# DakeQQ/Text-to-Speech-TTS-ONNX

Measured on AMD Instinct MI355X. Metric: audio_seconds_per_second, higher is better.
Workload: dtype f32

## Files before the change

text-to-speech-tts-onnx_amd/csrc/attention.hip:

```cpp
#include "common.h"
#include <functional>
#include <map>
#include <mutex>
#include <tuple>
#include "mfma.h"
#include "f5_kernels.h"
#include "x3_split.h"
#include "lds_dma.h"
#include <type_traits>
#include <string>
#include <algorithm>

namespace mi {

#define ATTN_XCD_MAP                                                                          \
    int bx_ = (int)blockIdx.x, by_ = (int)blockIdx.y;                                         \
    if (xmap) {                                                                               \
        const int l2 = bx_ + (int)gridDim.x * by_, slot = l2 >> 3;                            \
        by_ = (l2 & 7) + 8 * (slot / (int)gridDim.x);                                         \
        bx_ = slot % (int)gridDim.x;                                                          \
    }

#define ATTN_VARLEN_PROLOGUE                                                                  \
    const int NL = VARLEN ? lens[(bh / H) >> 1] : N;                                          \
// ... 390 lines not shown
}
__device__ __forceinline__ void attn_tr_use(attn_u2& d) {
#if defined(__HIP_DEVICE_COMPILE__)
    asm volatile("" : "+v"(d));
#endif
}
template <int N, int I = 0, typename F> __device__ __forceinline__ void attn_unroll(F&& f) {
    if constexpr (I < N) { f(std::integral_constant<int, I>{}); attn_unroll<N, I + 1>(f); }
}
template <int NP, int PLB, int S2> __device__ __forceinline__ void attn_v_tr_read(attn_u2 (&t)[2][NP][2], unsigned a0, unsigned a1) {
    attn_unroll<NP>([&](auto PL) {
        constexpr int pl = NP - 1 - decltype(PL)::value, o = pl * PLB + S2 * 16 * 128;
        attn_lds_rd64_tr16<o>(t[0][pl][0], a0); attn_lds_rd64_tr16<o + 8 * 128>(t[0][pl][1], a0);
        attn_lds_rd64_tr16<o>(t[1][pl][0], a1); attn_lds_rd64_tr16<o + 8 * 128>(t[1][pl][1], a1);
    });
}
#if defined(MI355TTS_ATTN_TRACE)
#define TSTAMP(v) do { __builtin_amdgcn_sched_barrier(0); asm volatile("s_memtime %0\n\ts_waitcnt lgkmcnt(0)" : "=s"(v) :: "memory"); __builtin_amdgcn_sched_barrier(0); } while (0)
#define TACC(k, t1, t0) tr_[k] += (t1) - (t0)
#else
#define TSTAMP(v) do { } while (0)
#define TACC(k, t1, t0) do { } while (0)
#endif
template <bool SPLIT2, bool KVP = false, int NP = 3, bool VARLEN = false, bool VROWS = false>
__global__ __launch_bounds__(256, NP == 2 ? 3 : 2) void attn_x3f_kernel(const float* __restrict__ q, const float* __restrict__ k,
                                                       const float* __restrict__ v, float* __restrict__ o, int H, int N,
                                                       float* __restrict__ ws, int* __restrict__ cnt,
                                                       unsigned char* __restrict__ o_planes, int o_np, int xmap = 0,
                                                       int cut1 = 0, int cut2 = 0, int cut3 = 0, const int* __restrict__ lens = nullptr) {
    ATTN_XCD_MAP
    static_assert(NP == 3 || (NP == 2 && KVP), "attn_x3f: the two-plane form reads pre-split K / V");
    static_assert(!VROWS || KVP, "attn_x3f: V as rows is a layout of the pre-split planes");
    using MF = std::conditional_t<NP == 3, Mfma<bf16>, Mfma<f16>>;
    using Frag = typename MF::Frag;
    constexpr int D = 64, KT = 64;
    constexpr int LDK = D + 8, LDV = VROWS ? D : KT + 4;
    constexpr int KPL = KT * LDK, VPL = VROWS ? KT * LDV : D * LDV;
    static_assert((NP * KPL * 2) % 16 == 0 && (VPL * 2) % 16 == 0, "attn_x3f: 16-byte aligned V planes");
    __shared__ __attribute__((aligned(16))) bf16 smem[NP * KPL + NP * VPL];
    static_assert(sizeof(smem) >= (2 * 32 * 64 + 2 * 64 * 2 + 4) * sizeof(float), "merge buffer fits the stage");
    bf16* Ks = smem;
    bf16* Vs = smem + NP * KPL;

    const int tid = threadIdx.x, wave = tid >> 6, lane = tid & 63, lr = lane & 31, hi = lane >> 5;
    const int bh = by_;
    ATTN_VARLEN_PROLOGUE
    const int q0 = SPLIT2 ? bx_ * 64 + (wave >> 1) * 32 : bx_ * 128 + wave * 32;
    const float* qb = q + (long)bh * N * D;
    const float* kb = k + (long)bh * N * D;
    const long vld = KVP ? (long)((N + 63) / 64 * 64) : (long)((N + 7) / 8 * 8);
    const float* vb = v + (long)bh * D * vld;
    const bf16* kpb = reinterpret_cast<const bf16*>(k) + (long)bh * NP * vld * D;
    const bf16* vpb = reinterpret_cast<const bf16*>(v) + (long)bh * NP * D * vld;

    auto split4 = [&](const float4 a, uint2& w1, uint2& w2, uint2& w3) __attribute__((always_inline)) {
        x3_split_pair(a.x, a.y, w1.x, w2.x, w3.x);
        x3_split_pair(a.z, a.w, w1.y, w2.y, w3.y);
    };
    auto split8 = [&](const float4 a, const float4 b, Frag& f1, Frag& f2, Frag& f3) __attribute__((always_inline)) {
        uint2 a1, a2, a3, b1, b2, b3;
        split4(a, a1, a2, a3); split4(b, b1, b2, b3);
        f1 = __builtin_bit_cast(Frag, u32x4{a1.x, a1.y, b1.x, b1.y});
// ... 94 lines not shown
                }
            }
        } else {
#pragma unroll
        for (int i = 0; i < 4; ++i) {
            const int vi = tid + i * 256;
            const int r = vi >> 4, c = vi & 15;
            uint2 w1, w2, w3;
            split4(kreg[i], w1, w2, w3);
            *reinterpret_cast<uint2*>(Ks + r * LDK + c * 4) = w1;
            *reinterpret_cast<uint2*>(Ks + KPL + r * LDK + c * 4) = w2;
            *reinterpret_cast<uint2*>(Ks + 2 * KPL + r * LDK + c * 4) = w3;
            split4(vreg[i], w1, w2, w3);
            *reinterpret_cast<uint2*>(Vs + r * LDV + c * 4) = w1;
            *reinterpret_cast<uint2*>(Vs + VPL + r * LDV + c * 4) = w2;
            *reinterpret_cast<uint2*>(Vs + 2 * VPL + r * LDV + c * 4) = w3;
        }
        }
    };

    unsigned vtr[2] = {0u, 0u};
    if constexpr (VROWS) {
        const int q4 = (lane >> 2) & 3;
        const unsigned a = lds_addr(Vs) + (4 * hi + q4) * (LDV * 2) + ((lane >> 4) & 1) * 32 + (lane & 3) * 8;
        vtr[0] = a + (q4 >> 1) * 64;
        vtr[1] = a + ((q4 >> 1) ^ 1) * 64;
    }
    f32x16 oacc[2];
#pragma unroll
    for (int r = 0; r < 16; ++r) { oacc[0][r] = 0.f; oacc[1][r] = 0.f; }
    float m_run = -INFINITY, l_run = 0.f;
#if defined(MI355TTS_ATTN_TRACE)
    unsigned long long tr_[8] = {0, 0, 0, 0, 0, 0, 0, 0}, ta_ = 0, tb_ = 0, tc_ = 0, td_ = 0, te_ = 0, tk_ = 0;
    TSTAMP(tk_);
#endif

    const int nstage_all = dead ? 0 : (NL + KT - 1) / KT;
    int st0 = (int)((long)blockIdx.z * nstage_all / gridDim.z);
    int nstage = (int)((long)(blockIdx.z + 1) * nstage_all / gridDim.z);
    if (cut1 > 0) {
        const int zz = (int)blockIdx.z, ZZ = (int)gridDim.z;
        st0 = zz == 0 ? 0 : zz == 1 ? cut1 : zz == 2 ? cut2 : cut3;
        nstage = zz + 1 == ZZ ? nstage_all : zz == 0 ? cut1 : zz == 1 ? cut2 : cut3;
    }
    if constexpr (VARLEN) { st0 = min(st0, nstage_all); nstage = min(nstage, nstage_all); }
    if (st0 < nstage) {
        load_regs(st0 * KT);
        store_lds();
        __syncthreads();
    }
    constexpr int TA[6] = {0, 1, 2, 0, 1, 0}, TB[6] = {2, 1, 0, 1, 0, 0};
    for (int st = st0; st < nstage; ++st) {
        if (st + 1 < nstage) load_regs((st + 1) * KT);
        auto tile = [&](int kt) {
            const int key0 = st * KT + kt * 32;
            TSTAMP(ta_);
            f32x16 sacc;
#pragma unroll
            for (int r = 0; r < 16; ++r) sacc[r] = 0.f;
#pragma unroll
            for (int ks = 0; ks < 4; ++ks) {
                Frag kf[NP];
#pragma unroll
                for (int pl = 0; pl < NP; ++pl)
                    kf[pl] = *reinterpret_cast<const Frag*>(Ks + pl * KPL + (kt * 32 + lr) * LDK + ks * 16 + hi * 8);
                if constexpr (NP == 3) {
#pragma unroll
                    for (int t = 0; t < 6; ++t) sacc = MF::mma(kf[TA[t]], qf3[ks][TB[t]], sacc);
                } else {
                    sacc = MF::mma(kf[1], qf3[ks][0], sacc);
                    sacc = MF::mma(kf[0], qf3[ks][1], sacc);
                    sacc = MF::mma(kf[0], qf3[ks][0], sacc);
                }
            }
            if (key0 + 32 > NL) {
#pragma unroll
                for (int r = 0; r < 16; ++r) {
                    const int key = key0 + (r & 3) + 8 * (r >> 2) + 4 * hi;
                    if (key >= NL) sacc[r] = -INFINITY;
                }
            }
            float mloc = -INFINITY;
#pragma unroll
            for (int r = 0; r < 16; ++r) mloc = fmaxf(mloc, sacc[r]);
            mloc = xor32_max(mloc);
#if defined(MI355TTS_ATTN_TRACE)
            { const float keep_ = mloc; asm volatile("" :: "v"(keep_)); }
#endif
            TSTAMP(tb_); TACC(0, tb_, ta_);
            float alpha = 1.f;
            if (!__all(mloc - m_run <= 8.0f)) {
                const float m_new = fmaxf(m_run, mloc);
                alpha = __builtin_amdgcn_exp2f(m_run - m_new);
                m_run = m_new;
#pragma unroll
                for (int r = 0; r < 16; ++r) { oacc[0][r] *= alpha; oacc[1][r] *= alpha; }
            }
            float p[16];
            float ls0 = 0.f, ls1 = 0.f;
#pragma unroll
            for (int r = 0; r < 16; r += 2) {
                float d0 = sacc[r] - m_run, d1 = sacc[r + 1] - m_run;
                asm("" : "+v"(d0)); asm("" : "+v"(d1));
                p[r] = __builtin_amdgcn_exp2f(d0); p[r + 1] = __builtin_amdgcn_exp2f(d1);
                ls0 += p[r]; ls1 += p[r + 1];
                asm("" : "+v"(ls0)); asm("" : "+v"(ls1));
            }
            float lsum = ls0 + ls1;
            lsum = xor32_sum(lsum);
            l_run = l_run * alpha + lsum;
#if defined(MI355TTS_ATTN_TRACE)
            { const float keep_ = l_run + p[0] + p[15]; asm volatile("" :: "v"(keep_)); }
#endif
            TSTAMP(tc_); TACC(1, tc_, tb_);
#pragma unroll
            for (int s2 = 0; s2 < 2; ++s2) {
                Frag pf[NP];
                if constexpr (NP == 3)
                    split8(float4{p[8 * s2], p[8 * s2 + 1], p[8 * s2 + 2], p[8 * s2 + 3]},
                           float4{p[8 * s2 + 4], p[8 * s2 + 5], p[8 * s2 + 6], p[8 * s2 + 7]}, pf[0], pf[1], pf[2]);
                else
                    split8p(float4{p[8 * s2], p[8 * s2 + 1], p[8 * s2 + 2], p[8 * s2 + 3]},
                            float4{p[8 * s2 + 4], p[8 * s2 + 5], p[8 * s2 + 6], p[8 * s2 + 7]}, pf[0], pf[1]);
                Frag vf[2][NP];
                if constexpr (VROWS) {
                    attn_u2 t[2][NP][2];
                    const unsigned a0 = vtr[0] + kt * (32 * LDV * 2), a1 = vtr[1] + kt * (32 * LDV * 2);
                    if (s2 == 0) attn_v_tr_read<NP, VPL * 2, 0>(t, a0, a1); else attn_v_tr_read<NP, VPL * 2, 1>(t, a0, a1);
                    attn_tr_wait();
#pragma unroll
                    for (int dt = 0; dt < 2; ++dt)
#pragma unroll
                        for (int pl = 0; pl < NP; ++pl) {
                            attn_tr_use(t[dt][pl][0]); attn_tr_use(t[dt][pl][1]);
                            vf[dt][pl] = __builtin_bit_cast(Frag, u32x4{t[dt][pl][0].x, t[dt][pl][0].y, t[dt][pl][1].x, t[dt][pl][1].y});
                        }
                } else {
#pragma unroll
                for (int dt = 0; dt < 2; ++dt)
#pragma unroll
                    for (int pl = 0; pl < NP; ++pl) {
                        const bf16* row = Vs + pl * VPL + (dt * 32 + lr) * LDV + kt * 32 + 16 * s2 + 4 * hi;
                        uint2 a2[2];
                        a2[0] = *reinterpret_cast<const uint2*>(row);
                        a2[1] = *reinterpret_cast<const uint2*>(row + 8);
                        vf[dt][pl] = __builtin_bit_cast(Frag, u32x4{a2[0].x, a2[0].y, a2[1].x, a2[1].y});
                    }
                }
                if constexpr (NP == 3) {
#pragma unroll
                    for (int t = 0; t < 6; ++t)
#pragma unroll
                        for (int dt = 0; dt < 2; ++dt) oacc[dt] = MF::mma(vf[dt][TA[t]], pf[TB[t]], oacc[dt]);
                } else {
                    oacc[0] = MF::mma(vf[0][1], pf[0], oacc[0]);
                    oacc[1] = MF::mma(vf[1][1], pf[0], oacc[1]);
                    oacc[0] = MF::mma(vf[0][0], pf[1], oacc[0]);
                    oacc[1] = MF::mma(vf[1][0], pf[1], oacc[1]);
                    oacc[0] = MF::mma(vf[0][0], pf[0], oacc[0]);
                    oacc[1] = MF::mma(vf[1][0], pf[0], oacc[1]);
                }
            }
            TSTAMP(td_); TACC(2, td_, tc_);
        };
        if constexpr (SPLIT2) {
            if (st * KT + (wave & 1) * 32 < NL) tile(wave & 1);
        } else {
#pragma unroll
            for (int kt = 0; kt < KT / 32; ++kt) {
                const int key0 = st * KT + kt * 32;
                if (key0 < NL) tile(kt);
            }
        }
        TSTAMP(ta_);
        __syncthreads();
        TSTAMP(tb_); TACC(3, tb_, ta_);
        if (st + 1 < nstage) {
            store_lds();
            TSTAMP(tc_); TACC(4, tc_, tb_);
            __syncthreads();
            TSTAMP(te_); TACC(5, te_, tc_);
        }
    }
#if defined(MI355TTS_ATTN_TRACE)
    TSTAMP(te_);
    if (blockIdx.x == 3 && blockIdx.y == 5 && (threadIdx.x & 63) == 0)
        printf("ATTN_TRACE z %d wave %d stages %d total %llu | S+max %llu exp %llu PV %llu bar1 %llu store %llu bar2 %llu\n", (int)blockIdx.z, wave, nstage - st0,
               te_ - tk_, tr_[0], tr_[1], tr_[2], tr_[3], tr_[4], tr_[5]);
#endif
    bool owner = true;
    constexpr int NG = SPLIT2 ? 2 : 4;
    int grp = wave;
    float* comb = reinterpret_cast<float*>(smem);
    float* stats = comb + 2 * 32 * 64;
    if constexpr (SPLIT2) {
        __syncthreads();
        grp = wave >> 1;
        owner = !(wave & 1);
        if (!owner) {
            stats[(grp * 64 + lane) * 2] = m_run; stats[(grp * 64 + lane) * 2 + 1] = l_run;
#pragma unroll
            for (int dt = 0; dt < 2; ++dt)
#pragma unroll
                for (int r = 0; r < 16; ++r) comb[((grp * 2 + dt) * 16 + r) * 64 + lane] = oacc[dt][r];
// ... 190 lines not shown
}

static int attn_pick_z(long units, long slot, int nstage, bool f32, int zmax, long ws_floats, long cnt_n) {
    auto fits = [&](int z) { return units * z * slot <= ws_floats && units <= cnt_n; };
    if (const int zf = opt(OPT_ATTN_Z_FORCE); zf > 0) return fits(zf) ? zf : 1;
    const int cus = device_cus();
    int Z = 1;
    double best = 1e30;
    for (int z = 1; z <= zmax; ++z) {
        if (z > 1 && (!fits(z) || nstage < 2 * z)) break;
        const double cost = (double)((units * z + cus - 1) / cus) / z * (1.0 + (f32 ? 0.09 : 0.06) * (z - 1));
        if (cost < best - 1e-9) { best = cost; Z = z; }
    }
    return Z;
}

struct AttnArgs { const AttnPlan& p; const void *q, *k, *v; void *o, *o_planes; int o_np; float* ws; int* cnt; const int* lens; hipStream_t s; };
using AttnThunk = void (*)(const AttnArgs&);
static dim3 attn_grid(const AttnPlan& p) { return dim3(p.grid[0], p.grid[1], p.grid[2]); }
template <typename T, bool SPLIT2, bool X3S, bool REFH, bool VARLEN> static void attn_go(const AttnArgs& a) {
    hipLaunchKernelGGL((attn_kernel<T, SPLIT2, X3S, REFH, VARLEN>), attn_grid(a.p), dim3(256), 0, a.s, (const T*)a.q, (const T*)a.k, (const T*)a.v,
                       (T*)a.o, a.p.H, a.p.N, a.ws, a.cnt, a.p.sscale, a.p.xmap, a.lens);
}
template <bool SPLIT2, bool KVP, int NP, bool VARLEN, bool VROWS> static void x3f_go(const AttnArgs& a) {
    hipLaunchKernelGGL((attn_x3f_kernel<SPLIT2, KVP, NP, VARLEN, VROWS>), attn_grid(a.p), dim3(256), 0, a.s, (const float*)a.q, (const float*)a.k,
                       (const float*)a.v, (float*)a.o, a.p.H, a.p.N, a.ws, a.cnt, (unsigned char*)a.o_planes, a.o_np, a.p.xmap, a.p.cut[0], a.p.cut[1],
                       a.p.cut[2], a.lens);
}
struct AttnEntry { const char* label; AttnThunk go[2][2]; };
#define ATTN_ROWS(T, SP, X3S, REFH) {{attn_go<T, SP, X3S, REFH, false>, nullptr}, {attn_go<T, SP, X3S, REFH, true>, nullptr}}
#define X3F_SPLITS(SP) {{x3f_go<SP, false, 3, false, false>, nullptr}, {x3f_go<SP, false, 3, true, false>, nullptr}}
#define X3F_PLANES(SP, NP) {{x3f_go<SP, true, NP, false, false>, x3f_go<SP, true, NP, false, true>}, {x3f_go<SP, true, NP, true, false>, x3f_go<SP, true, NP, true, true>}}
static const AttnEntry attn_table[ATTN_FORMS] = {
     {"attn_kernel<float, false>", ATTN_ROWS(float, false, false, false)},
     {"attn_kernel<float, true>", ATTN_ROWS(float, true, false, false)},
     {"attn_kernel<float, false, x3>", ATTN_ROWS(float, false, true, false)},
     {"attn_kernel<float, true, x3>", ATTN_ROWS(float, true, true, false)},
     {"attn_x3f_kernel<false>", X3F_SPLITS(false)},
     {"attn_x3f_kernel<true>", X3F_SPLITS(true)},
     {"attn_x3f_kernel<false, pre-split K V>", X3F_PLANES(false, 3)},
     {"attn_x3f_kernel<true, pre-split K V>", X3F_PLANES(true, 3)},
     {"attn_x3f_kernel<false, pre-split K V, fp16 pairs>", X3F_PLANES(false, 2)},
     {"attn_x3f_kernel<true, pre-split K V, fp16 pairs>", X3F_PLANES(true, 2)},
     {"attn_x3f_kernel<false, pre-split K V, fp16 pairs> + key slices", X3F_PLANES(false, 2)},
     {"attn_kernel<_Float16, false>", ATTN_ROWS(f16, false, false, false)},
     {"attn_kernel<_Float16, true>", ATTN_ROWS(f16, true, false, false)},
     {"attn_kernel<_Float16, false, reference-fp16 scores>", ATTN_ROWS(f16, false, false, true)},
     {"attn_kernel<_Float16, true, reference-fp16 scores>", ATTN_ROWS(f16, true, false, true)},
     {"attn_kernel<__bf16, false>", ATTN_ROWS(bf16, false, false, false)},
     {"attn_kernel<__bf16, true>", ATTN_ROWS(bf16, true, false, false)},
};
#undef ATTN_ROWS
#undef X3F_SPLITS
#undef X3F_PLANES

AttnPlan attention_plan(int BH, int H, int N, int dtype, bool caller_can_presplit_kv, bool has_lens, float ref_fp16_scale, long ws_floats,
                        long cnt_n) {
    MI_REQUIRE(ref_fp16_scale == 0.f || (dtype == MI_F16 && ref_fp16_scale > 0.f), "attention: the reference-fp16 score form needs f16 operands");
    MI_REQUIRE(H > 0 && BH % H == 0 && N > 0, "attention: bad shape");
    const bool f32 = dtype == MI_F32;
    AttnPlan p;
    p.kv = attention_kv_layout(N, dtype, caller_can_presplit_kv);
    p.varlen = has_lens; p.BH = BH; p.H = H; p.N = N; p.dtype = dtype;
    const int x3 = f32 ? opt_attn_x3() : 0, split = opt(OPT_ATTN_SPLIT);
    p.o_planes = f32 && x3 == 2;
    const int xm = (opt(OPT_ATTN_XCD_MAP) != 0 && BH % 8 == 0) ? 1 : 0;
    const int tiles = (N + ATTN_TILE - 1) / ATTN_TILE, tiles_split = (N + ATTN_TILE_SPLIT - 1) / ATTN_TILE_SPLIT, nstage = (N + ATTN_STAGE - 1) / ATTN_STAGE;
    if (ws_floats <= 0 || cnt_n <= 0) ws_floats = cnt_n = 0;
    const bool small = split && (long)tiles * BH < (f32 ? 1024 : 512) && N >= 64;
    int base, Z = 1;
    if (!f32) {
        base = dtype == MI_BF16 ? ATTN_BF16 : ref_fp16_scale != 0.f ? ATTN_F16_REF : ATTN_F16;
        if (base == ATTN_F16_REF) p.sscale = ref_fp16_scale; else p.xmap = xm;
        if (small) Z = attn_pick_z((long)tiles_split * BH, ATTN_SLOT_SPLIT, nstage, false, std::min((int)opt(OPT_ATTN_Z), (int)opt(OPT_ATTN_Z16)), ws_floats, cnt_n);
    } else {
        base = x3 == 1 ? ATTN_F32_QK_X3 : x3 != 2 ? ATTN_F32 : p.kv.kv_planes == 2 ? ATTN_X3F_PAIRS : p.kv.kv_planes ? ATTN_X3F_BF16X3 : ATTN_X3F;
        if (base == ATTN_X3F_PAIRS) p.xmap = xm;
        if (small && base == ATTN_X3F_PAIRS && split == 2) {
            const long units = (long)tiles * BH;
            AttnSlices sl;
            sl.Z = attn_pick_z(units, ATTN_SLOT, nstage, true, opt(OPT_ATTN_Z), ws_floats, cnt_n);
            auto fits = [&](int z) { return units * z * ATTN_SLOT <= ws_floats && units <= cnt_n; };
            if (opt(OPT_ATTN_LPT) && opt(OPT_ATTN_Z_FORCE) == 0 && ws_floats > 0) {
                int zm = std::min((int)opt(OPT_ATTN_Z), ATTN_MAX_SLICES);
                while (zm > 1 && !fits(zm)) --zm;
                sl = attn_pick_slices(units, nstage, 3 * device_cus(), zm);
                if (const AttnCuts& e = opt_attn_cuts(); e.n >= 1 && e.c[0] > 0 && e.c[0] < nstage && fits(e.n + 1)) {
                    sl.Z = e.n + 1; sl.cut[0] = e.c[0]; sl.cut[1] = e.n >= 2 ? e.c[1] : nstage; sl.cut[2] = e.n >= 3 ? e.c[2] : nstage;
                }
            }
            p.form = ATTN_X3F_PAIRS_SLICED;
            p.grid[0] = tiles; p.grid[1] = BH; p.grid[2] = sl.Z;
            p.cut[0] = sl.Z > 1 ? sl.cut[0] : 0; p.cut[1] = sl.cut[1]; p.cut[2] = sl.cut[2];
            p.label = attn_table[p.form].label;
            return p;
        }
        if (small) Z = attn_pick_z((long)tiles_split * BH, ATTN_SLOT_SPLIT, nstage, true, opt(OPT_ATTN_Z), ws_floats, cnt_n);
    }
    p.form = base + (small ? 1 : 0);
    p.grid[0] = small ? tiles_split : tiles; p.grid[1] = BH; p.grid[2] = Z;
    p.label = attn_table[p.form].label;
    return p;
}

void launch_attention(const AttnPlan& p, const void* q, const void* k, const void* v, void* o, void* o_planes, int o_np, float* ws, int* cnt,
                      const int* lens, hipStream_t s) {
    MI_REQUIRE(p.form >= 0 && p.form < ATTN_FORMS && p.BH > 0, "attention: no plan");
    MI_REQUIRE(o_np == 2 || o_np == 3, "attention: 2 or 3 output planes");
    MI_REQUIRE(!o_planes || p.o_planes, "attention: panel-plane output needs the fp32 split kernel");
    MI_REQUIRE(p.varlen == (lens != nullptr), "attention: the plan was made for a batch of the other kind (uniform / ragged)");
    MI_REQUIRE(p.grid[2] == 1 || (ws && cnt), "attention: the plan's key slices need the workspace it was told of");
    const AttnThunk go = attn_table[p.form].go[p.varlen ? 1 : 0][p.kv.v_rows ? 1 : 0];
    MI_REQUIRE(go, "attention: V as rows is a layout of the pre-split planes");
    const double esz = (double)dtype_size(p.dtype);
    ProfScope ps(FAM_ATTN, s, 4.0 * p.BH * p.N * 64.0 * esz, 4.0 * p.BH * (double)p.N * p.N * 64.0);
    prof_set_kernel(p.label);
    if (lens) prof_kernel_suffix(" + lengths");
    go({p, q, k, v, o, o_planes, o_np, ws, cnt, lens, s});
    MI_HIP(hipGetLastError());
}

}
```

text-to-speech-tts-onnx_amd/csrc/capi.hip:

```cpp
#include "common.h"
#include "bigvgan.h"
#include "f5.h"
#include "gpt.h"
#include "gpt_pick.h"
#include "cond.h"
#include <algorithm>
#include <mutex>
#include <exception>

using namespace mi;

struct mi_bigvgan { BigVGAN* impl; std::mutex mu; };
struct mi_f5 { F5* impl; std::mutex mu; };
struct mi_gpt { Gpt* impl; std::mutex mu; };
struct mi_cond { Cond* impl; std::mutex mu; };

template <typename F> static int guard(F&& f, bool exclusive = false) {
    try {
        options_init();
        std::shared_lock<std::shared_mutex> rd(option_lock(), std::defer_lock);
        std::unique_lock<std::shared_mutex> wr(option_lock(), std::defer_lock);
        if (exclusive) wr.lock(); else rd.lock();
        f();
        return MI_OK;
// ... 253 lines not shown

int mi_f5_tables(mi_f5* h, float* time_expand, float* delta_t) {
    return guard([&] {
        MI_REQUIRE(h && h->impl, "mi_f5_tables: null handle");
        std::lock_guard<std::mutex> lk_(h->mu);
        F5& e = *h->impl;
        if (time_expand) std::memcpy(time_expand, e.h_time_expand.data(), e.h_time_expand.size() * 4);
        if (delta_t) std::memcpy(delta_t, e.h_delta.data(), e.h_delta.size() * 4);
    });
}

int64_t mi_f5_info(mi_f5* h, const char* key) {
    int64_t v = -1;
    int rc = guard([&] {
        MI_REQUIRE(h && h->impl && key, "mi_f5_info: null handle / key");
        std::lock_guard<std::mutex> lk_(h->mu);
        F5& e = *h->impl;
        ArithScope as(e.arith);
        const std::string k(key);
        if (k == "f32_arithmetic") v = e.dtype != MI_F32 ? -1 : !gemm_x3_enabled() ? ARITH_NATIVE : (gemm_x3p_enabled() ? e.np : ARITH_BF16X3);
        else if (k == "saturation_events") v = e.sat_events;
        else if (k == "adaln_fold") v = (e.fold_built && e.cfg.ln_fold != 0) ? 1 : 0;
        else if (k == "attn_v_rows") v = attention_kv_layout(0, e.dtype, true).v_rows;
        else MI_REQUIRE(false, "mi_f5_info: unknown key");
    });
    return rc == MI_OK ? v : (int64_t)rc;
}

int mi_f5_preprocess(mi_f5* h, const int16_t* audio, int64_t L, const int32_t* text_ids, int64_t T, int64_t max_duration,
                     const float* noise_in, uint64_t seed, float* noise, float* rope_cos, float* rope_sin,
                     float* cat_mel_text, float* cat_mel_text_drop, int64_t* ref_signal_len, int mem) {
    return guard([&] {
        F5_CHECK(h, mem, "mi_f5_preprocess");
        F5& e = *h->impl;
        MI_REQUIRE(max_duration > 0 && max_duration <= e.cfg.max_len && T >= 0 && T < (1 << 20) && L > 0 && L < (1L << 31),
                   "mi_f5_preprocess: sizes");
        const int N = (int)max_duration;
        const int R = e.preprocess(1, audio, L, text_ids, (int)T, N, noise_in, seed, mem);
        hipStream_t s = e.stream;
        const size_t cd = e.cfg.cond_dim(), D = e.cfg.dim_head;
        copy_out(noise, e.d_noise.p, (size_t)N * e.cfg.mel * 4, mem, s);
        copy_out(rope_cos, e.rope_cos.p, (size_t)N * D * 4, mem, s);
        copy_out(rope_sin, e.rope_sin.p, (size_t)N * D * 4, mem, s);
        copy_out(cat_mel_text, e.d_cmt.p, (size_t)N * cd * 4, mem, s);
        copy_out(cat_mel_text_drop, e.d_cmtd.p, (size_t)N * cd * 4, mem, s);
        MI_HIP(hipStreamSynchronize(s));
// ... 821 lines not shown
```

text-to-speech-tts-onnx_amd/csrc/f5_kernels.h:

```cpp
#pragma once
#include "common.h"

namespace mi {

enum { NORM_LN_MOD = 0, NORM_LN_AFFINE = 1, NORM_L2 = 2 };
void launch_rownorm(int mode, const float* x, void* y, int out_dtype, const float* a, const float* b, long rows, int D,
                    float eps, hipStream_t s);
void launch_rownorm_len(int mode, const float* x, void* y, int out_dtype, const float* a, const float* b, int items, int Fmax, int D,
                        float eps, const int* lens, const long* offs, hipStream_t s);
void launch_rownorm_x3p(const float* x, void* planes, const float* a, const float* b, long rows, int D, float eps, hipStream_t s,
                        int np = 3, int* sat = nullptr);
void launch_ln_prologue(const float* x, void* aout, int a_dtype, int np, float* stats, const float* scale, long rows, int D, int* sat,
                        hipStream_t s);
void launch_ln_finalize(const float* partials, float* fin, long rows, int D, float eps, hipStream_t s);
void launch_ln_gather(const float* mod, long mod_ld, long col_scale, long col_shift, float* G, float* S, int steps, int D, hipStream_t s);
void launch_cast_to_f32(const void* src, int dtype, float* dst, long n, hipStream_t s);
void launch_absmax(const float* x, long n, unsigned* out_bits, hipStream_t s);
void launch_dwconv7(const float* x, float* y, const float* w, const float* bias, int B, int T, int C, hipStream_t s);
void launch_grn(float* y, float* ss_scratch, const float* gamma, const float* beta, int B, int T, int C, hipStream_t s);
void launch_text_gather(const int* ids, const float* emb, const float* pos, float* out, int U, int N, int C, hipStream_t s);
void launch_text_ids(const int32_t* in, int* out, int U, int T, int N, int vocab, int* err, hipStream_t s);
void launch_mask_rows(const int* ids, float* x, int V, int N, int C, hipStream_t s);
void launch_copy2d(const float* src, long lds_, void* dst, long ldd, long rows, int cols, int out_dtype, hipStream_t s);
void launch_pad_reflect(const int16_t* a, float* out, int U, long L, int half, hipStream_t s);
// ... 8 lines not shown
                           hipStream_t s, int parts = 1);
void launch_zero_pad_rows(void* x, long row_bytes, int items, int N, const int* len, int per, hipStream_t s);
void launch_sum_parts(const float* in, float* out, long rows, int M, int parts, hipStream_t s);

struct AttnKvLayout {
    int kv_planes = 0;
    long k_ld = 0;
    long v_ld = 0;
    int v_rows = 0;
};
AttnKvLayout attention_kv_layout(int N, int dtype, bool caller_can_presplit_kv);
enum AttnForm {
    ATTN_F32 = 0, ATTN_F32_QK_X3 = 2, ATTN_X3F = 4, ATTN_X3F_BF16X3 = 6, ATTN_X3F_PAIRS = 8,
    ATTN_X3F_PAIRS_SLICED = 10,
    ATTN_F16 = 11, ATTN_F16_REF = 13, ATTN_BF16 = 15, ATTN_FORMS = 17
};
constexpr int ATTN_TILE = 128, ATTN_TILE_SPLIT = 64, ATTN_STAGE = 64, ATTN_MAX_SLICES = 4;
constexpr long ATTN_SLOT_GROUP = 32 * 64 + 64 * 2, ATTN_SLOT_SPLIT = 2 * ATTN_SLOT_GROUP, ATTN_SLOT = 4 * ATTN_SLOT_GROUP;
constexpr long ATTN_WS_TILES = 2048;
struct AttnPlan {
    AttnKvLayout kv;
    bool o_planes = false;
    int form = ATTN_F32;
    bool varlen = false;
    int BH = 0, H = 0, N = 0, dtype = MI_F32;
    unsigned grid[3] = {1, 1, 1};
    int cut[3] = {0, 0, 0};
    int xmap = 0;
    float sscale = 1.f;
    const char* label = "";
};
AttnPlan attention_plan(int BH, int H, int N, int dtype, bool caller_can_presplit_kv, bool has_lens, float ref_fp16_scale, long ws_floats,
                        long cnt_n);
void launch_attention(const AttnPlan& plan, const void* q, const void* k, const void* v, void* o, void* o_planes, int o_np, float* ws,
                      int* cnt, const int* lens, hipStream_t s);

}
```

text-to-speech-tts-onnx_amd/csrc/options.h:

```cpp
#pragma once
#include <atomic>
#include <shared_mutex>

namespace mi {

#define MI_OPTIONS(X)                                                                                                   \
                                   \
    X(GEMM_BIG_TILE_MIN, "gemm_big_tile_min", "MI355TTS_BIG_TILE_MIN", ENV_INT, 160, STORE, 0, 0)                       \
    X(GEMM_N192_MIN, "gemm_n192_min", nullptr, ENV_INT, 160, STORE, 0, 0)                                               \
    X(GEMM_MID_TILE_MIN, "gemm_mid_tile_min", nullptr, ENV_INT, 160, STORE, 0, 0)                                       \
    X(GEMM_DMA3_K_MIN, "gemm_dma3_k_min", "MI355TTS_DMA3_K_MIN", ENV_INT, 2048, STORE, 0, 0)                            \
    X(GEMM_USE_DMA3, "gemm_use_dma3", "MI355TTS_NO_DMA3_GEMM", ENV_ONE_OFF, 1, BOOL, 0, 1)                              \
    X(GEMM_USE_DMA, "gemm_use_dma", "MI355TTS_NO_DMA_GEMM", ENV_ONE_OFF, 1, BOOL, 0, 1)                                 \
    X(GEMM_BIG_TILES, "gemm_big_tiles", "MI355TTS_NO_BIG_TILES", ENV_ONE_OFF, 1, BOOL, 0, 1)                            \
    X(GEMM_N192, "gemm_n192", "MI355TTS_NO_N192", ENV_ONE_OFF, 1, BOOL, 0, 1)                                           \
    X(GEMM_F32_DMA, "gemm_f32_dma", nullptr, ENV_INT, 1, BOOL, 0, 1)                                                    \
    X(GEMM_RING4, "gemm_ring4", "MI355TTS_NO_RING4", ENV_ONE_OFF, 1, BOOL, 0, 1)                                        \
    X(GEMM_RING4_MAX, "gemm_ring4_max", "MI355TTS_RING4_MAX", ENV_INT, 256, STORE, 0, 0)                                \
    X(GEMM_BUF, "gemm_buf", "MI355TTS_NO_BUF", ENV_ONE_OFF, 1, BOOL, 0, 1)                                              \
    X(GEMM_F32_SMALL, "gemm_f32_small", "MI355TTS_NO_F32_SMALL", ENV_ONE_OFF, 1, BOOL, 0, 1)                            \
    X(GEMM_F32_SMALL_MAX, "gemm_f32_small_max", "MI355TTS_F32_SMALL_MAX", ENV_INT, 1024, STORE, 0, 0)                   \
    X(GEMM_SMALL16_MAX, "gemm_small16_max", "MI355TTS_SMALL16_MAX", ENV_INT, 256, STORE, 0, 0)                          \
    X(GEMM_F32_N64_DMA, nullptr, "MI355TTS_F32_N64_DMA", ENV_INT, 1, STORE, 0, 0)                                       \
    X(GEMM_N64_DMA16, nullptr, "MI355TTS_N64_DMA16", ENV_INT, 0, STORE, 0, 0)  \
// ... 14 lines not shown
    X(GEMM_F32_N64_PAIRS, "gemm_f32_n64_pairs", nullptr, ENV_INT, 1, STORE, 0, 0)  \
    X(GEMM_F32_GCONV, "gemm_f32_gconv", nullptr, ENV_INT, 1, STORE, 0, 0)  \
    X(GEMM_X3P_NOALIGN, "gemm_x3p_noalign", "MI355TTS_X3P_NOALIGN", ENV_INT, 0, STORE, 0, 0)  \
    X(GEMM_X3P_GRID, "gemm_x3p_grid", "MI355TTS_X3P_GRID", ENV_INT, 0, STORE, 0, 0)  \
    X(GEMM_X3D, "gemm_x3d", "MI355TTS_X3D", ENV_INT, 1, STORE, 0, 0)                            \
    X(GEMM_X3D_MIN_EFF, "gemm_x3d_min_eff", "MI355TTS_X3D_MIN_EFF", ENV_INT, 90, STORE, 0, 0)  \
       \
    X(GEMM_PH8, "gemm_ph8", "MI355TTS_PH8", ENV_INT, 1, STORE, 0, 0)                                                    \
    X(GEMM_PH8_MIN_TILES, "gemm_ph8_min_tiles", "MI355TTS_PH8_MIN", ENV_INT, 200, STORE, 0, 0)                          \
    X(GEMM_PH8_ORDER, "gemm_ph8_order", "MI355TTS_PH8_ORDER", ENV_INT, 1, STORE, 0, 0)                                  \
     \
    X(GEMM_PH8_SPLIT_MAX, "gemm_ph8_split_max", "MI355TTS_PH8_SPLIT", ENV_INT, 2, CLAMP, 1, 4)                          \
    X(GEMM_PH8_SPLIT_MIN_NK, "gemm_ph8_split_min_nk", nullptr, ENV_INT, 24, STORE, 0, 0)                                \
                                                                            \
    X(GCONV_TWO_TAPS, "gconv_two_taps", "MI355TTS_GCONV2", ENV_ZERO_OFF, 1, BOOL, 0, 1)                                 \
    X(GCONV16, "gconv16", "MI355TTS_GCONV16", ENV_ZERO_OFF, 1, BOOL, 0, 1)                                              \
                                                                                         \
    X(ATTN_F32_X3, "attn_f32_x3", "MI355TTS_ATTN_X3", ENV_INT, 2, CLAMP, 0, 2)                                          \
    X(ATTN_F32_PLANES, "attn_f32_planes", "MI355TTS_ATTN_PLANES", ENV_INT, 2, REJECT, 2, 3)  \
    X(ATTN_SPLIT, "attn_split", "MI355TTS_ATTN_NO_SPLIT", ENV_ONE_OFF, 2, CLAMP, 0, 2)  \
    X(ATTN_XCD_MAP, "attn_xcd_map", nullptr, ENV_INT, 1, BOOL, 0, 1)  \
    X(ATTN_KV_PLANES, "attn_kv_planes", "MI355TTS_ATTN_KVP", ENV_INT, 1, BOOL, 0, 1)  \
    X(ATTN_V_ROWS, nullptr, "MI355TTS_ATTN_V_ROWS", ENV_ZERO_OFF, 1, BOOL, 0, 1)  \
    X(ATTN_LPT, "attn_lpt", "MI355TTS_ATTN_LPT", ENV_INT, 1, BOOL, 0, 1)  \
    X(ATTN_Z_FORCE, "attn_z_force", nullptr, ENV_INT, 0, CLAMP, 0, 4)  \
            \
    X(ATTN_Z, nullptr, "MI355TTS_ATTN_Z", ENV_INT, 4, CLAMP, 1, 4)                                                      \
    X(ATTN_Z16, nullptr, "MI355TTS_ATTN_Z16", ENV_INT, 1, CLAMP, 1, 4)                                                  \
    X(ATTN_CUTS, nullptr, "MI355TTS_ATTN_CUTS", ENV_CUTS, 0, STORE, 0, 0)  \
                                                                                              \
    X(GPT_MFMA_MIN, "gpt_mfma_min", nullptr, ENV_INT, 9, STORE, 0, 0)  \
    X(GPT_MFMA, nullptr, "MI355TTS_GPT_NO_MFMA", ENV_ONE_OFF, 1, BOOL, 0, 1)                                            \
                                                                    \
    X(BIGVGAN_STREAMS, "bigvgan_streams", nullptr, ENV_INT, 3, CLAMP, 1, 3)                                             \
    X(BV_SYNC, nullptr, "MI355TTS_BV_SYNC", ENV_ONE_ON, 0, BOOL, 0, 1)                                                  \
    X(AA_TILE, nullptr, "MI355TTS_AA_TILE", ENV_INT, 8192, STORE, 0, 0)    \
    X(AA_PIPE, nullptr, "MI355TTS_AA_PIPE", ENV_ZERO_OFF, 1, BOOL, 0, 1)                                                \
    X(AA_R, nullptr, "MI355TTS_AA_R", ENV_INT, 16, STORE, 0, 0)  \
    X(AACONV_LDS_MIN, nullptr, "MI355TTS_AACONV_LDS_MIN", ENV_INT, 0, STORE, 0, 0)

#define MI_OPT_ENUM(name, key, env, conv, dflt, policy, lo, hi) OPT_##name,
enum Opt : int { MI_OPTIONS(MI_OPT_ENUM) OPT_COUNT };

extern std::atomic<long> g_opt[OPT_COUNT];
static inline long opt(Opt o) { return g_opt[o].load(std::memory_order_relaxed); }

// ... 14 lines not shown
```

Measured before the change: 42.89.

## Stage pre-split K/V planes into LDS via buffer DMA ring in attention

Adds a DMA variant of the fp16-pair, V-as-rows attention kernel. It streams 32-key tiles of the pre-split K and V planes straight from global memory into a three-slot LDS ring using buffer-load-to-LDS, with an XOR swizzle on K rows so fragment reads avoid bank conflicts. This replaces the register load followed by an LDS store, and is meant to overlap the next tiles' fetch with compute while freeing registers and VALU work. It is on by default for the 128-query pair forms, and in exchange adds a barrier per 32-key tile and more LDS use.

```diff
diff --git a/text-to-speech-tts-onnx_amd/csrc/attention.hip b/text-to-speech-tts-onnx_amd/csrc/attention.hip
--- a/text-to-speech-tts-onnx_amd/csrc/attention.hip
+++ b/text-to-speech-tts-onnx_amd/csrc/attention.hip
@@ -436,7 +436,22 @@
 #define TSTAMP(v) do { } while (0)
 #define TACC(k, t1, t0) do { } while (0)
 #endif
-template <bool SPLIT2, bool KVP = false, int NP = 3, bool VARLEN = false, bool VROWS = false>
+constexpr int attn_k_swz(int row) { return (row >> 1) & 7; }
+constexpr bool attn_k_swz_ok() {
+    constexpr int G[2][16] = {{0, 1, 2, 3, 12, 13, 14, 15, 20, 21, 22, 23, 24, 25, 26, 27}, {4, 5, 6, 7, 8, 9, 10, 11, 16, 17, 18, 19, 28, 29, 30, 31}};
+    for (int g = 0; g < 2; ++g)
+        for (int c = 0; c < 8; ++c) {
+            unsigned seen = 0;
+            for (int i = 0; i < 16; ++i) {
+                const int slot = 8 * (G[g][i] & 1) + (c ^ attn_k_swz(G[g][i]));
+                if (seen >> slot & 1) return false;
+                seen |= 1u << slot;
+            }
+        }
+    return true;
+}
+static_assert(attn_k_swz_ok(), "attn_x3f DMA: the K fragment reads are conflict-free");
+template <bool SPLIT2, bool KVP = false, int NP = 3, bool VARLEN = false, bool VROWS = false, bool DMA = false>
 __global__ __launch_bounds__(256, NP == 2 ? 3 : 2) void attn_x3f_kernel(const float* __restrict__ q, const float* __restrict__ k,
                                                        const float* __restrict__ v, float* __restrict__ o, int H, int N,
                                                        float* __restrict__ ws, int* __restrict__ cnt,
@@ -451,7 +466,11 @@
     constexpr int LDK = D + 8, LDV = VROWS ? D : KT + 4;
     constexpr int KPL = KT * LDK, VPL = VROWS ? KT * LDV : D * LDV;
     static_assert((NP * KPL * 2) % 16 == 0 && (VPL * 2) % 16 == 0, "attn_x3f: 16-byte aligned V planes");
-    __shared__ __attribute__((aligned(16))) bf16 smem[NP * KPL + NP * VPL];
+    static_assert(!DMA || (KVP && VROWS && !SPLIT2 && NP == 2), "attn_x3f: LDS-DMA staging is built for the 128-query fp16-pair form with V as rows");
+    constexpr int RT = 32, RPL = RT * D * 2, RSLOT = 2 * NP * RPL, RING = 3;
+    constexpr int RPW = 2 * NP;
+    static_assert(!DMA || RING * RSLOT <= 65536, "attn_x3f DMA: the ring lies within 64 KB of LDS offsets");
+    __shared__ __attribute__((aligned(16))) bf16 smem[DMA ? RING * RSLOT / 2 : NP * KPL + NP * VPL];
     static_assert(sizeof(smem) >= (2 * 32 * 64 + 2 * 64 * 2 + 4) * sizeof(float), "merge buffer fits the stage");
     bf16* Ks = smem;
     bf16* Vs = smem + NP * KPL;
@@ -592,7 +611,7 @@
     unsigned vtr[2] = {0u, 0u};
     if constexpr (VROWS) {
         const int q4 = (lane >> 2) & 3;
-        const unsigned a = lds_addr(Vs) + (4 * hi + q4) * (LDV * 2) + ((lane >> 4) & 1) * 32 + (lane & 3) * 8;
+        const unsigned a = (DMA ? lds_addr(smem) + NP * RPL : lds_addr(Vs)) + (4 * hi + q4) * (LDV * 2) + ((lane >> 4) & 1) * 32 + (lane & 3) * 8;
         vtr[0] = a + (q4 >> 1) * 64;
         vtr[1] = a + ((q4 >> 1) ^ 1) * 64;
     }
@@ -614,132 +633,135 @@
         nstage = zz + 1 == ZZ ? nstage_all : zz == 0 ? cut1 : zz == 1 ? cut2 : cut3;
     }
     if constexpr (VARLEN) { st0 = min(st0, nstage_all); nstage = min(nstage, nstage_all); }
+    constexpr int TA[6] = {0, 1, 2, 0, 1, 0}, TB[6] = {2, 1, 0, 1, 0, 0};
+    const int kx = hi ^ attn_k_swz(lr);
+    auto tile = [&](int key0, int kt, unsigned slotb) {
+        TSTAMP(ta_);
+        f32x16 sacc;
+#pragma unroll
+        for (int r = 0; r < 16; ++r) sacc[r] = 0.f;
+#pragma unroll
+        for (int ks = 0; ks < 4; ++ks) {
+            Frag kf[NP];
+#pragma unroll
+            for (int pl = 0; pl < NP; ++pl)
+                if constexpr (DMA) kf[pl] = *reinterpret_cast<const Frag*>(reinterpret_cast<const char*>(smem) + slotb + pl * RPL + lr * (D * 2) + (((2 * ks) ^ kx) << 4));
+                else kf[pl] = *reinterpret_cast<const Frag*>(Ks + pl * KPL + (kt * 32 + lr) * LDK + ks * 16 + hi * 8);
+            if constexpr (NP == 3) {
+#pragma unroll
+                for (int t = 0; t < 6; ++t) sacc = MF::mma(kf[TA[t]], qf3[ks][TB[t]], sacc);
+            } else {
+                sacc = MF::mma(kf[1], qf3[ks][0], sacc);
+                sacc = MF::mma(kf[0], qf3[ks][1], sacc);
+                sacc = MF::mma(kf[0], qf3[ks][0], sacc);
+            }
+        }
+        if (key0 + 32 > NL) {
+#pragma unroll
+            for (int r = 0; r < 16; ++r) {
+                const int key = key0 + (r & 3) + 8 * (r >> 2) + 4 * hi;
+                if (key >= NL) sacc[r] = -INFINITY;
+            }
+        }
+        float mloc = -INFINITY;
+#pragma unroll
+        for (int r = 0; r < 16; ++r) mloc = fmaxf(mloc, sacc[r]);
+        mloc = xor32_max(mloc);
+#if defined(MI355TTS_ATTN_TRACE)
+        { const float keep_ = mloc; asm volatile("" :: "v"(keep_)); }
+#endif
+        TSTAMP(tb_); TACC(0, tb_, ta_);
+        float alpha = 1.f;
+        if (!__all(mloc - m_run <= 8.0f)) {
+            const float m_new = fmaxf(m_run, mloc);
+            alpha = __builtin_amdgcn_exp2f(m_run - m_new);
+            m_run = m_new;
+#pragma unroll
+            for (int r = 0; r < 16; ++r) { oacc[0][r] *= alpha; oacc[1][r] *= alpha; }
+        }
+        float p[16];
+        float ls0 = 0.f, ls1 = 0.f;
+#pragma unroll
+        for (int r = 0; r < 16; r += 2) {
+            float d0 = sacc[r] - m_run, d1 = sacc[r + 1] - m_run;
+            asm("" : "+v"(d0)); asm("" : "+v"(d1));
+            p[r] = __builtin_amdgcn_exp2f(d0); p[r + 1] = __builtin_amdgcn_exp2f(d1);
+            ls0 += p[r]; ls1 += p[r + 1];
+            asm("" : "+v"(ls0)); asm("" : "+v"(ls1));
+        }
+        float lsum = ls0 + ls1;
+        lsum = xor32_sum(lsum);
+        l_run = l_run * alpha + lsum;
+#if defined(MI355TTS_ATTN_TRACE)
+        { const float keep_ = l_run + p[0] + p[15]; asm volatile("" :: "v"(keep_)); }
+#endif
+        TSTAMP(tc_); TACC(1, tc_, tb_);
+#pragma unroll
+        for (int s2 = 0; s2 < 2; ++s2) {
+            Frag pf[NP];
+            if constexpr (NP == 3)
+                split8(float4{p[8 * s2], p[8 * s2 + 1], p[8 * s2 + 2], p[8 * s2 + 3]},
+                       float4{p[8 * s2 + 4], p[8 * s2 + 5], p[8 * s2 + 6], p[8 * s2 + 7]}, pf[0], pf[1], pf[2]);
+            else
+                split8p(float4{p[8 * s2], p[8 * s2 + 1], p[8 * s2 + 2], p[8 * s2 + 3]},
+                        float4{p[8 * s2 + 4], p[8 * s2 + 5], p[8 * s2 + 6], p[8 * s2 + 7]}, pf[0], pf[1]);
+            Frag vf[2][NP];
+            if constexpr (VROWS) {
+                attn_u2 t[2][NP][2];
+                const unsigned a0 = vtr[0] + (DMA ? slotb : kt * (32 * LDV * 2)), a1 = vtr[1] + (DMA ? slotb : kt * (32 * LDV * 2));
+                constexpr int PLB = DMA ? RPL : VPL * 2;
+                if (s2 == 0) attn_v_tr_read<NP, PLB, 0>(t, a0, a1); else attn_v_tr_read<NP, PLB, 1>(t, a0, a1);
+                attn_tr_wait();
+#pragma unroll
+                for (int dt = 0; dt < 2; ++dt)
+#pragma unroll
+                    for (int pl = 0; pl < NP; ++pl) {
+                        attn_tr_use(t[dt][pl][0]); attn_tr_use(t[dt][pl][1]);
+                        vf[dt][pl] = __builtin_bit_cast(Frag, u32x4{t[dt][pl][0].x, t[dt][pl][0].y, t[dt][pl][1].x, t[dt][pl][1].y});
+                    }
+            } else {
+#pragma unroll
+            for (int dt = 0; dt < 2; ++dt)
+#pragma unroll
+                for (int pl = 0; pl < NP; ++pl) {
+                    const bf16* row = Vs + pl * VPL + (dt * 32 + lr) * LDV + kt * 32 + 16 * s2 + 4 * hi;
+                    uint2 a2[2];
+                    a2[0] = *reinterpret_cast<const uint2*>(row);
+                    a2[1] = *reinterpret_cast<const uint2*>(row + 8);
+                    vf[dt][pl] = __builtin_bit_cast(Frag, u32x4{a2[0].x, a2[0].y, a2[1].x, a2[1].y});
+                }
+            }
+            if constexpr (NP == 3) {
+#pragma unroll
+                for (int t = 0; t < 6; ++t)
+#pragma unroll
+                    for (int dt = 0; dt < 2; ++dt) oacc[dt] = MF::mma(vf[dt][TA[t]], pf[TB[t]], oacc[dt]);
+            } else {
+                oacc[0] = MF::mma(vf[0][1], pf[0], oacc[0]);
+                oacc[1] = MF::mma(vf[1][1], pf[0], oacc[1]);
+                oacc[0] = MF::mma(vf[0][0], pf[1], oacc[0]);
+                oacc[1] = MF::mma(vf[1][0], pf[1], oacc[1]);
+                oacc[0] = MF::mma(vf[0][0], pf[0], oacc[0]);
+                oacc[1] = MF::mma(vf[1][0], pf[0], oacc[1]);
+            }
+        }
+        TSTAMP(td_); TACC(2, td_, tc_);
+    };
+    if constexpr (!DMA) {
     if (st0 < nstage) {
         load_regs(st0 * KT);
         store_lds();
         __syncthreads();
     }
-    constexpr int TA[6] = {0, 1, 2, 0, 1, 0}, TB[6] = {2, 1, 0, 1, 0, 0};
     for (int st = st0; st < nstage; ++st) {
         if (st + 1 < nstage) load_regs((st + 1) * KT);
-        auto tile = [&](int kt) {
-            const int key0 = st * KT + kt * 32;
-            TSTAMP(ta_);
-            f32x16 sacc;
-#pragma unroll
-            for (int r = 0; r < 16; ++r) sacc[r] = 0.f;
-#pragma unroll
-            for (int ks = 0; ks < 4; ++ks) {
-                Frag kf[NP];
-#pragma unroll
-                for (int pl = 0; pl < NP; ++pl)
-                    kf[pl] = *reinterpret_cast<const Frag*>(Ks + pl * KPL + (kt * 32 + lr) * LDK + ks * 16 + hi * 8);
-                if constexpr (NP == 3) {
-#pragma unroll
-                    for (int t = 0; t < 6; ++t) sacc = MF::mma(kf[TA[t]], qf3[ks][TB[t]], sacc);
-                } else {
-                    sacc = MF::mma(kf[1], qf3[ks][0], sacc);
-                    sacc = MF::mma(kf[0], qf3[ks][1], sacc);
-                    sacc = MF::mma(kf[0], qf3[ks][0], sacc);
-                }
-            }
-            if (key0 + 32 > NL) {
-#pragma unroll
-                for (int r = 0; r < 16; ++r) {
-                    const int key = key0 + (r & 3) + 8 * (r >> 2) + 4 * hi;
-                    if (key >= NL) sacc[r] = -INFINITY;
-                }
-            }
-            float mloc = -INFINITY;
-#pragma unroll
-            for (int r = 0; r < 16; ++r) mloc = fmaxf(mloc, sacc[r]);
-            mloc = xor32_max(mloc);
-#if defined(MI355TTS_ATTN_TRACE)
-            { const float keep_ = mloc; asm volatile("" :: "v"(keep_)); }
-#endif
-            TSTAMP(tb_); TACC(0, tb_, ta_);
-            float alpha = 1.f;
-            if (!__all(mloc - m_run <= 8.0f)) {
-                const float m_new = fmaxf(m_run, mloc);
-                alpha = __builtin_amdgcn_exp2f(m_run - m_new);
-                m_run = m_new;
-#pragma unroll
-                for (int r = 0; r < 16; ++r) { oacc[0][r] *= alpha; oacc[1][r] *= alpha; }
-            }
-            float p[16];
-            float ls0 = 0.f, ls1 = 0.f;
-#pragma unroll
-            for (int r = 0; r < 16; r += 2) {
-                float d0 = sacc[r] - m_run, d1 = sacc[r + 1] - m_run;
-                asm("" : "+v"(d0)); asm("" : "+v"(d1));
-                p[r] = __builtin_amdgcn_exp2f(d0); p[r + 1] = __builtin_amdgcn_exp2f(d1);
-                ls0 += p[r]; ls1 += p[r + 1];
-                asm("" : "+v"(ls0)); asm("" : "+v"(ls1));
-            }
-            float lsum = ls0 + ls1;
-            lsum = xor32_sum(lsum);
-            l_run = l_run * alpha + lsum;
-#if defined(MI355TTS_ATTN_TRACE)
-            { const float keep_ = l_run + p[0] + p[15]; asm volatile("" :: "v"(keep_)); }
-#endif
-            TSTAMP(tc_); TACC(1, tc_, tb_);
-#pragma unroll
-            for (int s2 = 0; s2 < 2; ++s2) {
-                Frag pf[NP];
-                if constexpr (NP == 3)
-                    split8(float4{p[8 * s2], p[8 * s2 + 1], p[8 * s2 + 2], p[8 * s2 + 3]},
-                           float4{p[8 * s2 + 4], p[8 * s2 + 5], p[8 * s2 + 6], p[8 * s2 + 7]}, pf[0], pf[1], pf[2]);
-                else
-                    split8p(float4{p[8 * s2], p[8 * s2 + 1], p[8 * s2 + 2], p[8 * s2 + 3]},
-                            float4{p[8 * s2 + 4], p[8 * s2 + 5], p[8 * s2 + 6], p[8 * s2 + 7]}, pf[0], pf[1]);
-                Frag vf[2][NP];
-                if constexpr (VROWS) {
-                    attn_u2 t[2][NP][2];
-                    const unsigned a0 = vtr[0] + kt * (32 * LDV * 2), a1 = vtr[1] + kt * (32 * LDV * 2);
-                    if (s2 == 0) attn_v_tr_read<NP, VPL * 2, 0>(t, a0, a1); else attn_v_tr_read<NP, VPL * 2, 1>(t, a0, a1);
-                    attn_tr_wait();
-#pragma unroll
-                    for (int dt = 0; dt < 2; ++dt)
-#pragma unroll
-                        for (int pl = 0; pl < NP; ++pl) {
-                            attn_tr_use(t[dt][pl][0]); attn_tr_use(t[dt][pl][1]);
-                            vf[dt][pl] = __builtin_bit_cast(Frag, u32x4{t[dt][pl][0].x, t[dt][pl][0].y, t[dt][pl][1].x, t[dt][pl][1].y});
-                        }
-                } else {
-#pragma unroll
-                for (int dt = 0; dt < 2; ++dt)
-#pragma unroll
-                    for (int pl = 0; pl < NP; ++pl) {
-                        const bf16* row = Vs + pl * VPL + (dt * 32 + lr) * LDV + kt * 32 + 16 * s2 + 4 * hi;
-                        uint2 a2[2];
-                        a2[0] = *reinterpret_cast<const uint2*>(row);
-                        a2[1] = *reinterpret_cast<const uint2*>(row + 8);
-                        vf[dt][pl] = __builtin_bit_cast(Frag, u32x4{a2[0].x, a2[0].y, a2[1].x, a2[1].y});
-                    }
-                }
-                if constexpr (NP == 3) {
-#pragma unroll
-                    for (int t = 0; t < 6; ++t)
-#pragma unroll
-                        for (int dt = 0; dt < 2; ++dt) oacc[dt] = MF::mma(vf[dt][TA[t]], pf[TB[t]], oacc[dt]);
-                } else {
-                    oacc[0] = MF::mma(vf[0][1], pf[0], oacc[0]);
-                    oacc[1] = MF::mma(vf[1][1], pf[0], oacc[1]);
-                    oacc[0] = MF::mma(vf[0][0], pf[1], oacc[0]);
-                    oacc[1] = MF::mma(vf[1][0], pf[1], oacc[1]);
-                    oacc[0] = MF::mma(vf[0][0], pf[0], oacc[0]);
-                    oacc[1] = MF::mma(vf[1][0], pf[0], oacc[1]);
-                }
-            }
-            TSTAMP(td_); TACC(2, td_, tc_);
-        };
         if constexpr (SPLIT2) {
-            if (st * KT + (wave & 1) * 32 < NL) tile(wave & 1);
+            if (st * KT + (wave & 1) * 32 < NL) tile(st * KT + (wave & 1) * 32, wave & 1, 0u);
         } else {
 #pragma unroll
             for (int kt = 0; kt < KT / 32; ++kt) {
                 const int key0 = st * KT + kt * 32;
-                if (key0 < NL) tile(kt);
+                if (key0 < NL) tile(key0, kt, 0u);
             }
         }
         TSTAMP(ta_);
@@ -750,6 +772,39 @@
             TSTAMP(tc_); TACC(4, tc_, tb_);
             __syncthreads();
             TSTAMP(te_); TACC(5, te_, tc_);
+        }
+    }
+    } else {
+        const int t0 = 2 * st0, t1 = min(2 * nstage, (NL + RT - 1) / RT);
+        __amdgpu_buffer_rsrc_t kd[NP], vd[NP];
+#pragma unroll
+        for (int pl = 0; pl < NP; ++pl) {
+            kd[pl] = buf_rsrc(kpb + (long)pl * vld * D, NL * (D * 2));
+            vd[pl] = buf_rsrc(vpb + (long)pl * vld * D, NL * (D * 2));
+        }
+        const int prow = 8 * wave + (lane >> 3), pch = lane & 7;
+        int koff = (t0 * RT + prow) * (D * 2) + ((pch ^ attn_k_swz(prow)) << 4);
+        int voff = (t0 * RT + prow) * (D * 2) + ((pch ^ ((prow & 2) << 1)) << 4);
+        const unsigned ring0 = lds_addr(smem) + (unsigned)__builtin_amdgcn_readfirstlane(wave) * 1024u;
+        auto issue = [&](int slot) {
+            const unsigned dst = ring0 + (unsigned)slot * RSLOT;
+#pragma unroll
+            for (int pl = 0; pl < NP; ++pl) dma16_buf(kd[pl], koff, dst + pl * RPL);
+#pragma unroll
+            for (int pl = 0; pl < NP; ++pl) dma16_buf(vd[pl], voff, dst + (NP + pl) * RPL);
+            koff += RPL; voff += RPL;
+        };
+        if (t0 < t1) issue(0);
+        if (t0 + 1 < t1) issue(1);
+        int slot = 0;
+        for (int t = t0; t < t1; ++t) {
+            TSTAMP(ta_);
+            if (t + 1 < t1) wait_vm<RPW * 1>(); else wait_vm<RPW * 0>();
+            __syncthreads();
+            TSTAMP(tb_); TACC(3, tb_, ta_);
+            if (t + 2 < t1) issue(slot == 0 ? 2 : slot - 1);
+            tile(t * RT, 0, (unsigned)slot * RSLOT);
+            slot = slot == 2 ? 0 : slot + 1;
         }
     }
 #if defined(MI355TTS_ATTN_TRACE)
@@ -986,12 +1041,13 @@
     hipLaunchKernelGGL((attn_kernel<T, SPLIT2, X3S, REFH, VARLEN>), attn_grid(a.p), dim3(256), 0, a.s, (const T*)a.q, (const T*)a.k, (const T*)a.v,
                        (T*)a.o, a.p.H, a.p.N, a.ws, a.cnt, a.p.sscale, a.p.xmap, a.lens);
 }
-template <bool SPLIT2, bool KVP, int NP, bool VARLEN, bool VROWS> static void x3f_go(const AttnArgs& a) {
-    hipLaunchKernelGGL((attn_x3f_kernel<SPLIT2, KVP, NP, VARLEN, VROWS>), attn_grid(a.p), dim3(256), 0, a.s, (const float*)a.q, (const float*)a.k,
+template <bool SPLIT2, bool KVP, int NP, bool VARLEN, bool VROWS, bool DMA = false> static void x3f_go(const AttnArgs& a) {
+    hipLaunchKernelGGL((attn_x3f_kernel<SPLIT2, KVP, NP, VARLEN, VROWS, DMA>), attn_grid(a.p), dim3(256), 0, a.s, (const float*)a.q, (const float*)a.k,
                        (const float*)a.v, (float*)a.o, a.p.H, a.p.N, a.ws, a.cnt, (unsigned char*)a.o_planes, a.o_np, a.p.xmap, a.p.cut[0], a.p.cut[1],
                        a.p.cut[2], a.lens);
 }
-struct AttnEntry { const char* label; AttnThunk go[2][2]; };
+struct AttnEntry { const char* label; AttnThunk go[2][2]; AttnThunk dma[2] = {nullptr, nullptr}; };
+#define X3F_DMA {x3f_go<false, true, 2, false, true, true>, x3f_go<false, true, 2, true, true, true>}
 #define ATTN_ROWS(T, SP, X3S, REFH) {{attn_go<T, SP, X3S, REFH, false>, nullptr}, {attn_go<T, SP, X3S, REFH, true>, nullptr}}
 #define X3F_SPLITS(SP) {{x3f_go<SP, false, 3, false, false>, nullptr}, {x3f_go<SP, false, 3, true, false>, nullptr}}
 #define X3F_PLANES(SP, NP) {{x3f_go<SP, true, NP, false, false>, x3f_go<SP, true, NP, false, true>}, {x3f_go<SP, true, NP, true, false>, x3f_go<SP, true, NP, true, true>}}
@@ -1004,9 +1060,9 @@
      {"attn_x3f_kernel<true>", X3F_SPLITS(true)},
      {"attn_x3f_kernel<false, pre-split K V>", X3F_PLANES(false, 3)},
      {"attn_x3f_kernel<true, pre-split K V>", X3F_PLANES(true, 3)},
-     {"attn_x3f_kernel<false, pre-split K V, fp16 pairs>", X3F_PLANES(false, 2)},
+     {"attn_x3f_kernel<false, pre-split K V, fp16 pairs>", X3F_PLANES(false, 2), X3F_DMA},
      {"attn_x3f_kernel<true, pre-split K V, fp16 pairs>", X3F_PLANES(true, 2)},
-     {"attn_x3f_kernel<false, pre-split K V, fp16 pairs> + key slices", X3F_PLANES(false, 2)},
+     {"attn_x3f_kernel<false, pre-split K V, fp16 pairs> + key slices", X3F_PLANES(false, 2), X3F_DMA},
      {"attn_kernel<_Float16, false>", ATTN_ROWS(f16, false, false, false)},
      {"attn_kernel<_Float16, true>", ATTN_ROWS(f16, true, false, false)},
      {"attn_kernel<_Float16, false, reference-fp16 scores>", ATTN_ROWS(f16, false, false, true)},
@@ -1017,6 +1073,7 @@
 #undef ATTN_ROWS
 #undef X3F_SPLITS
 #undef X3F_PLANES
+#undef X3F_DMA
 
 AttnPlan attention_plan(int BH, int H, int N, int dtype, bool caller_can_presplit_kv, bool has_lens, float ref_fp16_scale, long ws_floats,
                         long cnt_n) {
@@ -1027,6 +1084,7 @@
     p.kv = attention_kv_layout(N, dtype, caller_can_presplit_kv);
     p.varlen = has_lens; p.BH = BH; p.H = H; p.N = N; p.dtype = dtype;
     const int x3 = f32 ? opt_attn_x3() : 0, split = opt(OPT_ATTN_SPLIT);
+    const bool kv_dma = p.kv.kv_planes == 2 && p.kv.v_rows && opt(OPT_ATTN_KV_DMA) != 0;
     p.o_planes = f32 && x3 == 2;
     const int xm = (opt(OPT_ATTN_XCD_MAP) != 0 && BH % 8 == 0) ? 1 : 0;
     const int tiles = (N + ATTN_TILE - 1) / ATTN_TILE, tiles_split = (N + ATTN_TILE_SPLIT - 1) / ATTN_TILE_SPLIT, nstage = (N + ATTN_STAGE - 1) / ATTN_STAGE;
@@ -1054,6 +1112,7 @@
                 }
             }
             p.form = ATTN_X3F_PAIRS_SLICED;
+            p.kv_dma = kv_dma;
             p.grid[0] = tiles; p.grid[1] = BH; p.grid[2] = sl.Z;
             p.cut[0] = sl.Z > 1 ? sl.cut[0] : 0; p.cut[1] = sl.cut[1]; p.cut[2] = sl.cut[2];
             p.label = attn_table[p.form].label;
@@ -1062,6 +1121,7 @@
         if (small) Z = attn_pick_z((long)tiles_split * BH, ATTN_SLOT_SPLIT, nstage, true, opt(OPT_ATTN_Z), ws_floats, cnt_n);
     }
     p.form = base + (small ? 1 : 0);
+    p.kv_dma = kv_dma && base == ATTN_X3F_PAIRS && !small;
     p.grid[0] = small ? tiles_split : tiles; p.grid[1] = BH; p.grid[2] = Z;
     p.label = attn_table[p.form].label;
     return p;
@@ -1074,8 +1134,8 @@
     MI_REQUIRE(!o_planes || p.o_planes, "attention: panel-plane output needs the fp32 split kernel");
     MI_REQUIRE(p.varlen == (lens != nullptr), "attention: the plan was made for a batch of the other kind (uniform / ragged)");
     MI_REQUIRE(p.grid[2] == 1 || (ws && cnt), "attention: the plan's key slices need the workspace it was told of");
-    const AttnThunk go = attn_table[p.form].go[p.varlen ? 1 : 0][p.kv.v_rows ? 1 : 0];
-    MI_REQUIRE(go, "attention: V as rows is a layout of the pre-split planes");
+    const AttnThunk go = p.kv_dma ? attn_table[p.form].dma[p.varlen ? 1 : 0] : attn_table[p.form].go[p.varlen ? 1 : 0][p.kv.v_rows ? 1 : 0];
+    MI_REQUIRE(go, p.kv_dma ? "attention: LDS-DMA staging is a form of the 128-query fp16-pair kernels" : "attention: V as rows is a layout of the pre-split planes");
     const double esz = (double)dtype_size(p.dtype);
     ProfScope ps(FAM_ATTN, s, 4.0 * p.BH * p.N * 64.0 * esz, 4.0 * p.BH * (double)p.N * p.N * 64.0);
     prof_set_kernel(p.label);
diff --git a/text-to-speech-tts-onnx_amd/csrc/capi.hip b/text-to-speech-tts-onnx_amd/csrc/capi.hip
--- a/text-to-speech-tts-onnx_amd/csrc/capi.hip
+++ b/text-to-speech-tts-onnx_amd/csrc/capi.hip
@@ -299,6 +299,10 @@
         else if (k == "saturation_events") v = e.sat_events;
         else if (k == "adaln_fold") v = (e.fold_built && e.cfg.ln_fold != 0) ? 1 : 0;
         else if (k == "attn_v_rows") v = attention_kv_layout(0, e.dtype, true).v_rows;
+        else if (k == "attn_kv_dma") {
+            const int H = e.cfg.heads;
+            v = attention_plan(2 * H, H, 1024, e.dtype, true, false, 0.f, ATTN_WS_TILES * ATTN_MAX_SLICES * ATTN_SLOT_SPLIT, ATTN_WS_TILES).kv_dma ? 1 : 0;
+        }
         else MI_REQUIRE(false, "mi_f5_info: unknown key");
     });
     return rc == MI_OK ? v : (int64_t)rc;
diff --git a/text-to-speech-tts-onnx_amd/csrc/f5_kernels.h b/text-to-speech-tts-onnx_amd/csrc/f5_kernels.h
--- a/text-to-speech-tts-onnx_amd/csrc/f5_kernels.h
+++ b/text-to-speech-tts-onnx_amd/csrc/f5_kernels.h
@@ -54,6 +54,7 @@
     AttnKvLayout kv;
     bool o_planes = false;
     int form = ATTN_F32;
+    bool kv_dma = false;
     bool varlen = false;
     int BH = 0, H = 0, N = 0, dtype = MI_F32;
     unsigned grid[3] = {1, 1, 1};
diff --git a/text-to-speech-tts-onnx_amd/csrc/options.h b/text-to-speech-tts-onnx_amd/csrc/options.h
--- a/text-to-speech-tts-onnx_amd/csrc/options.h
+++ b/text-to-speech-tts-onnx_amd/csrc/options.h
@@ -60,6 +60,7 @@
     X(ATTN_XCD_MAP, "attn_xcd_map", nullptr, ENV_INT, 1, BOOL, 0, 1)  \
     X(ATTN_KV_PLANES, "attn_kv_planes", "MI355TTS_ATTN_KVP", ENV_INT, 1, BOOL, 0, 1)  \
     X(ATTN_V_ROWS, nullptr, "MI355TTS_ATTN_V_ROWS", ENV_ZERO_OFF, 1, BOOL, 0, 1)  \
+    X(ATTN_KV_DMA, nullptr, "MI355TTS_ATTN_KV_DMA", ENV_ZERO_OFF, 1, BOOL, 0, 1)  \
     X(ATTN_LPT, "attn_lpt", "MI355TTS_ATTN_LPT", ENV_INT, 1, BOOL, 0, 1)  \
     X(ATTN_Z_FORCE, "attn_z_force", nullptr, ENV_INT, 0, CLAMP, 0, 4)  \
             \
```

New measurement: 43.12 (median of 6 runs). No clear change (+0.5%).
